# arhix52/Strelka

Measured on AMD Instinct MI355X. Metric: Mray/s, higher is better.
Workload: dtype f32; 1 GPU; kitchen stand-in (SURVEY 8d C3): 1724134 unique triangles, 2022 instances of 153 meshes, 4 rect + 1 distant light, 60/25/10/5 % diffuse/glossy/metal/glass; resolution=1920x1080, bounces=4, spp=64, tile=32, world_size=1, parallelism=single GPU, rays_per_frame=839862650

## Files before the change

strelka_amd/build.py:

```python
import os
import subprocess

HERE = os.path.dirname(os.path.abspath(__file__))
ROOT = os.path.dirname(HERE)
LIB = os.environ.get("SKH_LIB") or os.path.join(HERE, "libstrelka_hip.so")
SRC = os.path.join(HERE, "csrc", "strelka_hip.hip")
DEPS = [SRC] + [os.path.join(HERE, "csrc", f) for f in ("skh_device.h", "skh_bvh.h", "skh_env.h", "skh_emit.h", "skh_blend.h", "skh_adapt.h", "skh_aov.h", "skh_denoise.h", "skh_temporal.h", "skh_variance.h", "skh_lshape.h", "skh_kernels.h", "skh_shade_body.inc", "skh_trace_body.inc", "skh_libm.h", "skh_host.h", "skh_stale.h", "skh_accel.inc", "skh_probes.inc")] + [
    os.path.join(ROOT, "include", "strelka_hip.h"), os.path.abspath(__file__)]
FLAGS = ["-O3", "--offload-arch=gfx950", "-ffp-contract=off", "-fno-slp-vectorize", "-mllvm", "-amdgpu-sched-strategy=max-ilp",
         "-fPIC", "-shared", "-std=c++17"]


def hipcc():
    for c in (os.environ.get("HIPCC"), "/opt/rocm/bin/hipcc", "hipcc"):
        if c and (os.path.isabs(c) and os.path.exists(c) or not os.path.isabs(c)):
            return c
    return "hipcc"


def needs_build():
    if os.environ.get("SKH_LIB") and os.path.exists(LIB):
        return False
    return not os.path.exists(LIB) or any(os.path.getmtime(d) > os.path.getmtime(LIB) for d in DEPS)


def build_variant(out_path, defines, verbose=False):
    cmd = [hipcc()] + FLAGS + ["-D" + d for d in defines] + ["-o", out_path, SRC]
    if verbose:
        print(" ".join(cmd))
    subprocess.check_call(cmd)
    return out_path


def build(force=False, verbose=False):
    if not force and not needs_build():
        return LIB
    import fcntl

    with open(LIB + ".lock", "w") as lock:
        fcntl.flock(lock, fcntl.LOCK_EX)
        try:
            if force or needs_build():
                tmp = "%s.tmp.%d" % (LIB, os.getpid())
                cmd = [hipcc()] + FLAGS + ["-o", tmp, SRC]
                if verbose:
                    print(" ".join(cmd))
                subprocess.check_call(cmd)
                os.replace(tmp, LIB)
        finally:
            fcntl.flock(lock, fcntl.LOCK_UN)
    return LIB


HOST_DIR = os.path.join(HERE, "host")
HOST_LIB = os.path.join(HOST_DIR, "liboka_hip.so")
HOST_TEST = os.path.join(HOST_DIR, "host_test")


def build_host(force=False, verbose=False):
    build(force=False, verbose=verbose)
# ... 40 lines not shown
```

strelka_amd/csrc/skh_host.h:

```cpp
#pragma once
#include "../../include/strelka_hip.h"
#include "skh_kernels.h"
#include "skh_stale.h"

#include <string>
#include <utility>
#include <vector>

typedef struct ncclComm* ncclComm_t;
using namespace skh;

namespace
{
struct DevBuf
{
    void* p = nullptr;
    size_t bytes = 0;
    DevBuf() = default;
    DevBuf(const DevBuf&) = delete;
    DevBuf& operator=(const DevBuf&) = delete;
    DevBuf(DevBuf&& o) noexcept : p(o.p), bytes(o.bytes)
    {
        o.p = nullptr;
        o.bytes = 0;
    }
    DevBuf& operator=(DevBuf&& o) noexcept
    {
        if (this != &o)
        {
            reset();
            p = o.p, bytes = o.bytes;
            o.p = nullptr, o.bytes = 0;
        }
        return *this;
    }
    ~DevBuf()
    {
        reset();
    }
    void reset()
    {
        if (p)
            (void)hipFree(p);
        p = nullptr;
        bytes = 0;
    }
    template <typename T>
    T* as() const
    {
        return reinterpret_cast<T*>(p);
    }
};

enum KernelClass
{
// ... 32 lines not shown
        uint32_t* hOverflow = nullptr;
        std::string err;
    } dev;

    struct MultiGpu
    {
        ncclComm_t comm = nullptr;
        int world = 1, rank = 0;
        DevBuf dTileSend, dScatterXY;
    } multi;

    struct Scene
    {
        std::vector<skh_mesh> meshes;
        std::vector<skh_curve> curves;
        std::vector<uint32_t> curveVertexCounts;
        std::vector<skh_instance> instances;
        std::vector<int32_t> lightTypes;
        uint32_t nVerts = 0, nIndices = 0, nPoints = 0, nInstances = 0, nLights = 0, nMaterials = 0;
        DevBuf dVerts, dIndices, dMeshes, dPoints, dRadii, dInstances, dLights, dMaterials, dHairConst;
        uint64_t geomSig = 0, curveSig = 0;
        DevBuf dTexels, dTexDesc;
        uint32_t nTextures = 0;
        bool hasHairMaterial = false;
    } scene;

    struct Options
    {
        bool countTraversal = false, timing = false;
        int overlap = 1;
        uint32_t speculateAsync = 1;
        uint32_t speculateGrow = 2;
        uint32_t speculateMax = 8;
        uint32_t envNee = 1, emitNee = 1;
        uint32_t cutoutRounds = 8;
        uint32_t aovBand = 1u << 22;
        int32_t fetchChunk = -1;
        uint32_t wavesPerCU = 28;
        uint32_t wavesPerCUShadow = 28;
        uint32_t wavesPerCUShadowWorld = 32;
        uint32_t wavesPerCUWorld = 32;
        uint32_t smallWavesClosest = 0, smallWavesShadow = 0;
        uint32_t fetchMinClosestSmall = 48;
        uint32_t smallWavesFirst = 0, smallWavesLast = 0;
        int tailSplit = 1;
        uint32_t fetchMinClosest = 32 , fetchMinShadow = 48;
        bool fetchMinClosestSet = false;
        uint32_t curveFetchMinClosest = 16, curveFetchMinShadow = 16 , curveNodeBreakClosest = 20, curveNodeBreakShadow = 20;
        uint32_t nodeBreakClosest = 32, nodeBreakShadow = 28;
        uint32_t worldCurveMin = 32;
        uint32_t curveMin = 48;
        uint32_t leafMin = 16;
        uint32_t subframeBatch = 0;
        bool worldKernel = true;
        uint32_t reinsertRounds = 8;
        uint32_t reinsertCurveRounds = 4;
        uint32_t reinsertMinSize = 0;
        uint32_t plocTop = 0;
        bool tightInstanceBoxes = true;
        uint32_t curveLeaf = 1;
        uint32_t splitPairs = 0;
        uint32_t curveMerge = 1;
        uint32_t curveSegNode = 0;
        uint32_t curveStrandMajor = 0;
        uint32_t curveSplit = 4;
        uint32_t tlasBuild = 1;
        uint32_t tlasOpen = 1;
        uint32_t bakeWorld = 4, bakeSmallTris = 64, bakeBudgetMTris = 64;
        uint32_t mortonBits = 10;
        uint32_t leafLines = 0;
        uint32_t mergeLightProxies = 0;
        int32_t directRecords = -1;
        uint32_t compactHits = 1;
        uint32_t leafMaxTris = 2;
        uint32_t buildQuality = 1;
    } opt;

    struct Accel
    {
        bool built = false;
        DevBuf dTriNodes, dTris, dSegNodes, dSegs, dTlasNodes, dTlasInst, dDevInst, dTravInst;
        DevBuf dShadeTris, dShadeInst;
        DevBuf dCurveSegBase, dSegStartAll;
        int tlasRoot = SKH_REF_INVALID;
        int worldRoot = SKH_REF_INVALID, lightRoot = SKH_REF_INVALID;
        uint32_t nTris = 0, nSegs = 0;
        uint32_t nTriSlots = 0;
        uint32_t hierNodes = 0;
        uint32_t numTlasLeaves = 0;
        uint32_t curveSplitBuilt = 1;
        uint32_t numWorldCurves = 0;
        int worldCurveRoot[SKH_WORLD_CURVES];
        uint32_t worldCurveInst[SKH_WORLD_CURVES];
        uint32_t worldCurveMerged = 0;
        uint32_t worldCurveIdentLast = 0;
        uint32_t numMergedCurveInst = 0;
        std::vector<uint8_t> baked;
        uint32_t nBakedTris = 0, nBakedInst = 0;
        LightBox lightBox = { { -INFINITY, -INFINITY, -INFINITY }, { INFINITY, INFINITY, INFINITY } };
        uint32_t nShadeRecords = 0;
        uint32_t directRecords = 1;
        uint32_t hitPrimRange = 0;
        skh_build_info buildInfo = {};
        double msBuild = 0.0;
        bool refitReady = false;
        DevBuf dTriOrder, dTriMeshK, dTriLocalK, dWInstK, dWFirstK, dTriNodeBox;
// ... 17 lines not shown
        std::vector<uint32_t> tlasLevelStart;
    } accel;

    struct Environment
    {
        DevBuf dTexels, dColCdf, dRowCdf;
        uint32_t w = 0, h = 0;
        float scale[3] = { 1.0f, 1.0f, 1.0f }, w2e[9] = { 1.0f, 0.0f, 0.0f, 0.0f, 1.0f, 0.0f, 0.0f, 0.0f, 1.0f };
        double sumW = 0.0, msBuild = 0.0;
    } env;

    struct Emitters
    {
        std::vector<float> emission;
        bool stale = false;
        DevBuf dEntries, dCdf, dGuide, dLe, dInstOffset;
        uint32_t count = 0, instances = 0, guideBits = 0;
        double sumW = 0.0, msBuild = 0.0;
    } emit;

    struct MaterialTextures
    {
        std::vector<skh_material_textures> table;
        DevBuf dTable;
    } mtex;

    struct Cut
    {
        std::vector<skh_material_cutout> cutouts;
        DevBuf dCutouts, dStats, dQ[2], dHits, dShadowQ[2], dShadowHits[2];
        bool stale = false;
        uint32_t activeMaterials = 0, instances = 0;
        std::vector<skh_material_blend> blends;
        DevBuf dBlend;
        uint32_t blendActiveMaterials = 0, blendInstances = 0;
    } cut;

    struct LightShapes
    {
        std::vector<skh_light_shape> table;
        DevBuf dTable;
        bool stale = false;
        uint32_t discs = 0, cones = 0;
    } lshape;

    struct Frame
    {
        uint32_t width = 0, height = 0, tileSize = 32, tileShift = 5, numTiles = 0, numSlots = 0;
        std::vector<uint32_t> tileXY;
        bool customTiles = false;
        DevBuf dTileXY, dAccum, dDiffuse, dSpecular, dDiffCnt, dSpecCnt, dSums, dPath, dRayQ[2], dHits, dShadowQ, dContrib, dCounts, dOvf, dOvf2, dScratchImage;
        DevBuf dRaygenBase;
        uint32_t raygenBlocksPerSub = 0, raygenValidPerSub = 0;
        std::vector<uint32_t> chunkValid;
        uint32_t queueConstBits[2] = { 0, 0 };
        bool queueConstFilled = false;
        uint32_t batchCapacity = 1;
        uint32_t queueRegion = 64;
        uint32_t traceBlocks = 0;
    } frame;

    struct Speculation
    {
        bool valid = false;
        skh_frame_params params;
        uint32_t count = 0, consumed = 0, lastBatch = 1, streak = 0;
        skh_frame_params last;
        bool haveLast = false;
        uint64_t passRadiance = 0, passShadow = 0;
        uint32_t buf = 0;
        bool nextInFlight = false;
        skh_frame_params nextParams;
        uint32_t nextCount = 0;
        unsigned long long statsMark[2] = { 0, 0 };
        DevBuf dPathB;
        uint32_t pathBStride = 0;
        uint64_t discardedRadiance = 0, discardedShadow = 0;
        uint32_t discardedSubframes = 0;
    } spec;

    struct Adaptive
    {
        bool on = false;
        skh_adaptive cfg = {};
        bool ready = false;
        uint32_t delivered = 0;
        uint32_t checks = 0, activeTiles = 0, raygenValid = 0;
        uint64_t pixelObs = 0, pixelObsSaved = 0;
        std::vector<uint32_t> frozenAt;
        DevBuf dTileXYRender, dRaygenBaseRender, dState, dTileQ, dFrozenAt;
    } adapt;

    struct Timing
    {
        std::vector<TimedSpan> spans;
        std::vector<hipEvent_t> eventPool;
        size_t eventsUsed = 0;
        double msClass[KC_COUNT] = { 0, 0, 0, 0, 0, 0, 0 };
        uint32_t launches[KC_COUNT] = { 0, 0, 0, 0, 0, 0, 0 };
        DevBuf dStats;
        uint32_t stackOverflows = 0;
    } timing;

    struct Aov
    {
        skh_aov_info info = {};
    } aov;

    struct Denoiser
    {
        DevBuf dColor[2], dG0, dG1;
        skh_denoise_info info = {};
    } dn;

    struct Temporal
    {
        skh_temporal_info info = {};
    } tp;

    struct Moments
    {
        skh_moments_info info = {};
    } mo;
    struct VarianceDenoiser
    {
        skh_vdenoise_info info = {};
    } vd;
};

static inline void touched(skh_context* c, skh_stale::Input in)
{
    using namespace skh_stale;
    bool* flag[D_COUNT] = {};
    flag[D_ACCEL_BUILT] = &c->accel.built, flag[D_REFIT_READY] = &c->accel.refitReady, flag[D_UPDATE_READY] = &c->accel.updateReady;
    flag[D_VERTS_EDITED] = &c->accel.vertsEdited, flag[D_CURVE_POINTS_EDITED] = &c->accel.curvePointsEdited;
    flag[D_EMIT_STALE] = &c->emit.stale, flag[D_CUT_STALE] = &c->cut.stale, flag[D_LSHAPE_STALE] = &c->lshape.stale;
    apply(in, flag);
}

#define SKH_TRY(ctx, expr)                                                                                              \
// ... 41 lines not shown
```

strelka_amd/csrc/skh_kernels.h:

```cpp
#pragma once
#include "skh_bvh.h"
#include "skh_env.h"
#include "skh_emit.h"
#include "skh_blend.h"

namespace skh
{

struct DevInstance
{
    float w2o[12];
    int rootRef;
    uint32_t mask;
    uint32_t type;
    uint32_t pad;
};
struct HostInstance
{
    float o2w[12];
    uint32_t type, geom, material, light;
};

#define SKH_WORLD_CURVES 2
#define SKH_SEG_STRIDE 8
// ... 503 lines not shown
    __syncthreads();
    if (threadIdx.x == 0)
    {
        uint32_t tot = 0;
        for (uint32_t w = 0; w < nw; ++w)
        {
            const uint32_t cnt = s_wave[w];
            s_wave[w] = tot;
            tot += cnt;
        }
        s_wave[SKH_COMPACT_MAX_WAVES] = tot ? atomicAdd(counter, tot) : 0u;
    }
    __syncthreads();
    const uint32_t r = s_wave[SKH_COMPACT_MAX_WAVES] + s_wave[wave] + rank_below(m);
    __syncthreads();
    return r;
}
SKH_DI void block_compact2(bool emitA, uint32_t* counterA, bool emitB, uint32_t* counterB, uint32_t* s_wave2, uint32_t& ia, uint32_t& ib)
{
    const uint32_t lane = threadIdx.x & 63u, wave = threadIdx.x >> 6, nw = blockDim.x >> 6;
    const unsigned long long ma = __ballot(emitA), mb = __ballot(emitB);
    uint32_t* sa = s_wave2;
    uint32_t* sb = s_wave2 + SKH_COMPACT_MAX_WAVES + 1;
    if (lane == 0)
    {
        sa[wave] = (uint32_t)__popcll(ma);
        sb[wave] = (uint32_t)__popcll(mb);
    }
    __syncthreads();
    if (threadIdx.x == 0 || threadIdx.x == 64)
    {
        uint32_t* sw = threadIdx.x == 0 ? sa : sb;
        uint32_t tot = 0;
        for (uint32_t w = 0; w < nw; ++w)
        {
            const uint32_t cnt = sw[w];
            sw[w] = tot;
            tot += cnt;
        }
        sw[SKH_COMPACT_MAX_WAVES] = tot ? atomicAdd(threadIdx.x == 0 ? counterA : counterB, tot) : 0u;
    }
    if (nw == 1 && threadIdx.x == 0)
    {
        uint32_t tot = sb[0];
        sb[0] = 0;
        sb[SKH_COMPACT_MAX_WAVES] = tot ? atomicAdd(counterB, tot) : 0u;
    }
    __syncthreads();
    ia = sa[SKH_COMPACT_MAX_WAVES] + sa[wave] + rank_below(ma);
    ib = sb[SKH_COMPACT_MAX_WAVES] + sb[wave] + rank_below(mb);
}

__global__ void __launch_bounds__(512) k_raygen(FrameP fp, const uint32_t* __restrict__ tileXY, uint32_t sampleOffset, RayQ rq,
                                               uint32_t* __restrict__ counter, PathS ps, const uint32_t* __restrict__ blockBase,
                                               uint32_t blocksPerSub, uint32_t validPerSub)
{
    __shared__ uint32_t s_wave[SKH_COMPACT_MAX_WAVES + 1];
    const uint32_t sub = blockIdx.x / blocksPerSub, bi = blockIdx.x - sub * blocksPerSub;
    const uint32_t slot = bi * blockDim.x + threadIdx.x;
    const uint32_t path = sub * fp.numSlots + slot;
    uint32_t px = 0, py = 0;
    const bool active = sub < fp.batch && slot < fp.numSlots && slot_to_pixel(fp, tileXY, slot, px, py);
    v3 o = mk3(0.0f), d = mk3(0.0f);
    if (active)
    {
        const Sampler s = init_sampler(px, py, fp.subframeIndex + sampleOffset + sub, fp.sppTotal, 52u);
        generate_camera_ray(px, py, fp.width, fp.height, fp.clipToView, fp.viewToWorld, sampler_random(s, DIM_PIXEL_X),
                            sampler_random(s, DIM_PIXEL_Y), o, d);
        ps.rad()[path] = make_float4(0.0f, 0.0f, 0.0f, 0.0f);
        reinterpret_cast<uint32_t*>(ps.base)[path + 7 * (size_t)ps.stride] = 0u;
    }
    const uint32_t lane = threadIdx.x & 63u, wave = threadIdx.x >> 6;
    const unsigned long long m = __ballot(active);
    if (lane == 0)
        s_wave[wave] = (uint32_t)__popcll(m);
    __syncthreads();
    uint32_t before = 0;
    for (uint32_t w = 0; w < wave; ++w)
        before += s_wave[w];
    const uint32_t dense = sub * validPerSub + blockBase[bi] + before + rank_below(m);
    const uint32_t total = validPerSub * fp.batch;
    const uint32_t per = (((total + SKH_SHARDS - 1u) / SKH_SHARDS) + 63u) & ~63u;
    const uint32_t shard = per ? dense / per : 0u;
    const uint32_t idx = shard * rq.region + (dense - shard * per);
    if (blockIdx.x == 0 && threadIdx.x < SKH_SHARDS)
        counter[threadIdx.x * SKH_COUNT_STRIDE] = min(per, total - min(total, threadIdx.x * per));
    if (active)
    {
        rq.plane(0)[idx] = o.x;
        rq.plane(1)[idx] = o.y;
        rq.plane(2)[idx] = o.z;
        rq.plane(3)[idx] = d.x;
        rq.plane(4)[idx] = d.y;
        rq.plane(5)[idx] = d.z;
        rq.ids()[idx] = path;
    }
}

__global__ void __launch_bounds__(256) k_gather_shade_tris(const uint8_t* __restrict__ verts, const uint32_t* __restrict__ indices,
                                                          const uint4* __restrict__ meshes, const uint32_t* __restrict__ meshTriBase,
                                                          uint32_t nMeshes, uint32_t nTris, float4* __restrict__ out)
{
    const uint32_t g = blockIdx.x * blockDim.x + threadIdx.x;
    if (g >= nTris)
        return;
    uint32_t lo = 0, hi = nMeshes;
    while (hi - lo > 1u)
    {
        const uint32_t mid = (lo + hi) >> 1;
        if (meshTriBase[mid] <= g)
            lo = mid;
        else
            hi = mid;
    }
    const uint4 me = meshes[lo];
    const uint32_t t = g - meshTriBase[lo];
    float4 v0[3], v1[3];
#pragma unroll
    for (uint32_t k = 0; k < 3u; ++k)
    {
        const uint32_t idx = indices[me.x + 3u * t + k];
        const float4* v = reinterpret_cast<const float4*>(verts + (size_t)(me.z + idx) * 32);
        v0[k] = v[0], v1[k] = v[1];
    }
    float4* o = out + 6 * (size_t)g;
#pragma unroll
    for (uint32_t k = 0; k < 3u; ++k)
        o[k] = make_float4(v0[k].x, v0[k].y, v0[k].z, v1[k].x);
    o[3] = make_float4(v0[0].w, v0[1].w, v0[2].w, v1[0].y);
    o[4] = make_float4(v1[1].y, v1[2].y, 0.0f, 0.0f);
    o[5] = make_float4(0.0f, 0.0f, 0.0f, 0.0f);
}

// ... 926 lines not shown
```

strelka_amd/csrc/strelka_hip.hip:

```cpp
#include "../../include/strelka_hip.h"
#include "skh_kernels.h"

#include <dlfcn.h>
typedef struct ncclComm* ncclComm_t;
typedef struct
{
    char internal[128];
} ncclUniqueId;
typedef enum
{
    ncclSuccess = 0
} ncclResult_t;
typedef enum
{
    ncclFloat = 7
} ncclDataType_t;

#include <algorithm>
#include <chrono>
#include <cmath>
#include <cstdio>
#include <cstring>
#include <mutex>
#include <string>
// ... 468 lines not shown
{
    const uint32_t nMeshes = (uint32_t)c->scene.meshes.size();
    std::vector<uint32_t> base(nMeshes + 1u, 0u);
    uint64_t total = 0;
    for (uint32_t m = 0; m < nMeshes; ++m)
    {
        total += c->scene.meshes[m].index_count / 3u;
        base[m + 1] = (uint32_t)std::min<uint64_t>(total, 0xffffffffull);
    }
    const uint32_t nTris = base[nMeshes];
    c->accel.nShadeRecords = nTris;
    if (total >= SKH_PRIM_DIRECT)
    {
        c->dev.err = "skh_build_accel: more than 2^31 - 1 triangles (the primitive word of a hit keeps its top bit for SKH_PRIM_DIRECT)";
        return SKH_INVALID_ARGUMENT;
    }
    SKH_CHECK(dev_alloc(c, c->accel.dShadeTris, std::max<size_t>(96, (size_t)nTris * 96)));
    if (nTris)
    {
        DevBuf dBase;
        SKH_CHECK(dev_upload(c, dBase, base.data(), sizeof(uint32_t) * base.size()));
        k_gather_shade_tris<<<(nTris + 255u) / 256u, 256, 0, c->dev.stream>>>(c->scene.dVerts.as<uint8_t>(), c->scene.dIndices.as<uint32_t>(), c->scene.dMeshes.as<uint4>(),
                                                                         dBase.as<uint32_t>(), nMeshes, nTris, c->accel.dShadeTris.as<float4>());
        SKH_TRY(c, hipStreamSynchronize(c->dev.stream));
    }
    std::vector<skh_instance> inst = c->scene.instances;
    for (skh_instance& i : inst)
        if (i.type == SKH_INSTANCE_MESH)
            i.light_id = i.geom_id < nMeshes ? base[i.geom_id] : 0u;
    if (inst.empty())
        inst.resize(1);
    return dev_upload(c, c->accel.dShadeInst, inst.data(), sizeof(skh_instance) * inst.size());
}

#include "skh_accel.inc"


static size_t frame_count_words(const skh_context* c);

static void raygen_tables(const skh_context* c, const uint32_t* frozenAt, std::vector<uint32_t>& base, uint32_t& total)
{
    const uint32_t blocks = (c->frame.numSlots + 511u) / 512u, chunks = (uint32_t)c->frame.chunkValid.size(), shift2 = 2 * c->frame.tileShift;
    base.assign(std::max(1u, blocks), 0u);
    total = 0;
    for (uint32_t b = 0; b < blocks; ++b)
    {
        base[b] = total;
        for (uint32_t j = b * 8u; j < std::min(chunks, (b + 1) * 8u); ++j)
            if (!frozenAt || frozenAt[(j * 64u) >> shift2] == 0u)
                total += c->frame.chunkValid[j];
    }
}

static skh_status alloc_frame(skh_context* c)
{
    const uint32_t T = c->frame.tileSize;
    if (!c->frame.customTiles)
    {
        c->frame.tileXY.clear();
        for (uint32_t y = 0; y < c->frame.height; y += T)
            for (uint32_t x = 0; x < c->frame.width; x += T)
            {
                c->frame.tileXY.push_back(x);
                c->frame.tileXY.push_back(y);
            }
    }
    c->frame.numTiles = (uint32_t)(c->frame.tileXY.size() / 2);
    c->frame.numSlots = c->frame.numTiles * T * T;
    c->frame.batchCapacity = c->opt.subframeBatch ? c->opt.subframeBatch : std::min(64u, std::max(1u, (1u << 27) / std::max(1u, c->frame.numSlots)));
    const size_t N1 = std::max(1u, c->frame.numSlots);
    const size_t N = N1 * c->frame.batchCapacity;
    c->frame.queueRegion = (uint32_t)((((N + SKH_SHARDS - 1) / SKH_SHARDS) + 63) & ~(size_t)63);
    const size_t NQ = (size_t)SKH_SHARDS * c->frame.queueRegion;
    SKH_CHECK(dev_upload(c, c->frame.dTileXY, c->frame.tileXY.data(), sizeof(uint32_t) * c->frame.tileXY.size()));
    {
        auto compact = [](uint32_t x) {
            x &= 0x55555555u;
            x = (x ^ (x >> 1)) & 0x33333333u;
            x = (x ^ (x >> 2)) & 0x0f0f0f0fu;
            x = (x ^ (x >> 4)) & 0x00ff00ffu;
            x = (x ^ (x >> 8)) & 0x0000ffffu;
            return x;
        };
        const uint32_t shift2 = 2 * c->frame.tileShift, mask = (1u << shift2) - 1u;
        c->frame.chunkValid.assign(c->frame.numSlots / 64u, 0u);
        for (uint32_t j = 0; j < c->frame.numSlots / 64u; ++j)
        {
            const uint32_t tile = (j * 64u) >> shift2, m = (j * 64u) & mask;
            const uint32_t x0 = c->frame.tileXY[2 * tile] + compact(m), y0 = c->frame.tileXY[2 * tile + 1] + compact(m >> 1);
            uint32_t n = 0;
            for (uint32_t k = 0; k < 64u; ++k)
                n += (x0 + compact(k) < c->frame.width && y0 + compact(k >> 1) < c->frame.height) ? 1u : 0u;
            c->frame.chunkValid[j] = n;
        }
        std::vector<uint32_t> base;
        raygen_tables(c, nullptr, base, c->frame.raygenValidPerSub);
        c->frame.raygenBlocksPerSub = (uint32_t)((c->frame.numSlots + 511u) / 512u);
        SKH_CHECK(dev_upload(c, c->frame.dRaygenBase, base.data(), sizeof(uint32_t) * base.size()));
    }
    c->adapt.ready = false;
    SKH_CHECK(dev_alloc(c, c->frame.dAccum, sizeof(float4) * N1));
    SKH_CHECK(dev_alloc(c, c->frame.dDiffuse, sizeof(float4) * N1));
    SKH_CHECK(dev_alloc(c, c->frame.dSpecular, sizeof(float4) * N1));
    SKH_CHECK(dev_alloc(c, c->frame.dDiffCnt, sizeof(uint16_t) * N1));
    SKH_CHECK(dev_alloc(c, c->frame.dSpecCnt, sizeof(uint16_t) * N1));
    SKH_CHECK(dev_alloc(c, c->frame.dSums, sizeof(float) * 11 * N1));
    SKH_CHECK(dev_alloc(c, c->frame.dPath, sizeof(float) * SKH_PATH_FLOATS * N));
    SKH_CHECK(dev_alloc(c, c->frame.dRayQ[0], sizeof(float) * 9 * NQ));
    SKH_CHECK(dev_alloc(c, c->frame.dRayQ[1], sizeof(float) * 9 * NQ));
// ... 972 lines not shown
    if (!a || !std::isfinite(a->threshold) || a->threshold < 0.0f || !std::isfinite(a->dark_level) || !(a->dark_level > 0.0f) || a->min_samples < 2u ||
        a->interval < 1u || a->reserved[0] || a->reserved[1] || a->reserved[2] || a->reserved[3])
        return SKH_INVALID_ARGUMENT;
    return SKH_OK;
}

skh_status skh_set_adaptive(skh_context* c, const skh_adaptive* a)
{
    if (!c || (a && skh_adaptive_check(a) != SKH_OK))
    {
        if (c)
            c->dev.err = "skh_set_adaptive: threshold finite and >= 0, dark_level finite and > 0, min_samples >= 2, interval >= 1, reserved words 0";
        return SKH_INVALID_ARGUMENT;
    }
    (void)hipSetDevice(c->dev.device);
    spec_drop(c);
    c->adapt.on = a != nullptr;
    if (a)
        c->adapt.cfg = *a;
    else
    {
        SKH_TRY(c, hipStreamSynchronize(c->dev.stream));
        c->adapt = skh_context::Adaptive();
    }
    return SKH_OK;
}

static inline bool adapt_applies(const skh_context* c, const skh_frame_params& p)
{
    return c->adapt.on && p.enable_accumulation != 0 && p.debug == 0;
}

static skh_status adapt_prepare(skh_context* c, const skh_frame_params& p)
{
    skh_context::Adaptive& ad = c->adapt;
    if (ad.ready && p.subframe_index != 0)
        return SKH_OK;
    const size_t N1 = std::max(1u, c->frame.numSlots), nt = std::max(1u, c->frame.numTiles);
    const size_t baseBytes = sizeof(uint32_t) * std::max(1u, c->frame.raygenBlocksPerSub);
    SKH_CHECK(dev_alloc(c, c->adapt.dTileXYRender, sizeof(uint32_t) * 2 * nt));
    SKH_CHECK(dev_alloc(c, c->adapt.dRaygenBaseRender, baseBytes));
    SKH_CHECK(dev_alloc(c, c->adapt.dState, sizeof(float4) * N1));
    SKH_CHECK(dev_alloc(c, c->adapt.dTileQ, sizeof(float) * nt));
    SKH_CHECK(dev_alloc(c, c->adapt.dFrozenAt, sizeof(uint32_t) * nt));
    SKH_TRY(c, hipMemcpyAsync(c->adapt.dTileXYRender.p, c->frame.dTileXY.p, sizeof(uint32_t) * 2 * c->frame.numTiles, hipMemcpyDeviceToDevice, c->dev.stream));
    SKH_TRY(c, hipMemcpyAsync(c->adapt.dRaygenBaseRender.p, c->frame.dRaygenBase.p, baseBytes, hipMemcpyDeviceToDevice, c->dev.stream));
    SKH_TRY(c, hipMemsetAsync(c->adapt.dState.p, 0, sizeof(float4) * N1, c->dev.stream));
    SKH_TRY(c, hipMemsetAsync(c->adapt.dTileQ.p, 0, sizeof(float) * nt, c->dev.stream));
    SKH_TRY(c, hipMemsetAsync(c->adapt.dFrozenAt.p, 0, sizeof(uint32_t) * nt, c->dev.stream));
    ad.frozenAt.assign(c->frame.numTiles, 0u);
    ad.delivered = ad.checks = 0;
    ad.activeTiles = c->frame.numTiles;
    ad.raygenValid = c->frame.raygenValidPerSub;
    ad.pixelObs = ad.pixelObsSaved = 0;
    ad.ready = true;
    return SKH_OK;
}

static inline uint32_t adapt_to_next_check(const skh_context* c)
{
    const skh_context::Adaptive& ad = c->adapt;
    if (ad.delivered < ad.cfg.min_samples)
        return ad.cfg.min_samples - ad.delivered;
    return ad.cfg.interval - (ad.delivered - ad.cfg.min_samples) % ad.cfg.interval;
}

static void frame_geometry(const skh_context* c, FrameP& fp)
{
    fp.width = c->frame.width, fp.height = c->frame.height, fp.tileSize = c->frame.tileSize, fp.tileShift = c->frame.tileShift, fp.numTiles = c->frame.numTiles, fp.numSlots = c->frame.numSlots;
}

static FrameP adapt_frame(const skh_context* c, const skh_frame_params& p)
{
    FrameP fp;
    memset(&fp, 0, sizeof(fp));
    memcpy(fp.exposure, p.exposure, sizeof(fp.exposure));
    frame_geometry(c, fp);
    return fp;
}

static skh_status adapt_after_pass(skh_context* c, const skh_frame_params& p, uint32_t launches)
{
    skh_context::Adaptive& ad = c->adapt;
    ad.delivered += launches;
    ad.pixelObs += (uint64_t)ad.raygenValid * launches;
    ad.pixelObsSaved += (uint64_t)(c->frame.raygenValidPerSub - ad.raygenValid) * launches;
    if (ad.delivered < ad.cfg.min_samples || (ad.delivered - ad.cfg.min_samples) % ad.cfg.interval != 0u || c->frame.numTiles == 0u)
        return SKH_OK;
    const float thr2 = ad.cfg.threshold * ad.cfg.threshold;
    {
        SpanGuard g(c, KC_ACCUM);
        k_adapt_tiles<<<c->frame.numTiles, 256, 0, c->dev.stream>>>(adapt_frame(c, p), c->adapt.dTileXYRender.as<uint32_t>(), c->adapt.dState.as<float4>(), ad.delivered, thr2,
                                                          ad.cfg.dark_level, c->adapt.dTileQ.as<float>(), c->adapt.dFrozenAt.as<uint32_t>());
    }
    ad.checks++;
    SKH_TRY(c, hipMemcpyAsync(ad.frozenAt.data(), c->adapt.dFrozenAt.p, sizeof(uint32_t) * c->frame.numTiles, hipMemcpyDeviceToHost, c->dev.stream));
    SKH_TRY(c, hipStreamSynchronize(c->dev.stream));
    uint32_t active = 0;
    for (uint32_t t = 0; t < c->frame.numTiles; ++t)
        active += ad.frozenAt[t] == 0u ? 1u : 0u;
    if (active != ad.activeTiles)
    {
        std::vector<uint32_t> base;
        raygen_tables(c, ad.frozenAt.data(), base, ad.raygenValid);
        SKH_TRY(c, hipMemcpyAsync(c->adapt.dRaygenBaseRender.p, base.data(), sizeof(uint32_t) * base.size(), hipMemcpyHostToDevice, c->dev.stream));
        SKH_TRY(c, hipStreamSynchronize(c->dev.stream));
        ad.activeTiles = active;
    }
    return SKH_OK;
}

static void adapt_fill(skh_context* c, const skh_frame_params& p, void* d_image)
{
    if (!d_image || c->adapt.activeTiles == c->frame.numTiles || c->frame.numSlots == 0u)
        return;
    SpanGuard g(c, KC_ACCUM);
    k_adapt_fill<<<(c->frame.numSlots + 255) / 256, 256, 0, c->dev.stream>>>(adapt_frame(c, p), c->frame.dTileXY.as<uint32_t>(), c->adapt.dFrozenAt.as<uint32_t>(),
                                                                 c->frame.dAccum.as<float4>(), reinterpret_cast<float4*>(d_image));
}

skh_status skh_get_adaptive_info(skh_context* c, skh_adaptive_info* out)
{
    if (!c || !out)
        return SKH_INVALID_ARGUMENT;
    const skh_context::Adaptive& ad = c->adapt;
    memset(out, 0, sizeof(*out));
    out->enabled = ad.on ? 1u : 0u;
    out->tiles = c->frame.numTiles;
    out->active_tiles = c->frame.numTiles;
    if (!ad.on || !ad.ready)
        return SKH_OK;
    out->active_tiles = ad.activeTiles;
    out->checks = ad.checks;
    uint32_t lo = 0xffffffffu, hi = 0;
    for (uint32_t t = 0; t < c->frame.numTiles; ++t)
    {
        const uint32_t n = ad.frozenAt[t] ? ad.frozenAt[t] : ad.delivered;
        lo = std::min(lo, n), hi = std::max(hi, n);
    }
    out->min_observations = c->frame.numTiles ? lo : 0u;
    out->max_observations = hi;
    out->pixel_observations = ad.pixelObs;
    out->pixel_observations_saved = ad.pixelObsSaved;
    return SKH_OK;
}

struct RenderPlan
{
    uint32_t batch = 1;
    bool trace = true;
    uint32_t finalFirst = 0, finalCount = 0xffffffffu;
    uint32_t pathSel = 0;
    bool finalize = true;
    hipStream_t finStream = nullptr;
    bool adaptive = false;
};

struct RenderPass
{
    FrameP fp;
// ... 116 lines not shown
        t.smallGrid = smallGrids ? ((b + 1 == rp.rounds && (c->opt.smallWavesLast || (!c->opt.smallWavesShadow && !c->accel.nSegs))) ? (c->opt.smallWavesLast ? c->opt.smallWavesLast : 20u) : c->opt.smallWavesShadow ? c->opt.smallWavesShadow : (c->accel.nSegs ? 16u : 12u)) * (uint32_t)c->dev.numCUs : 0u;
        const CutRounds cr{ { rp.cutSQ[0], rp.cutSQ[1] }, rp.cutSH0, rp.cutSH1, nullptr, rp.cutOn ? words + c->opt.cutoutRounds * SKH_CUT_WORDS : nullptr, rp.NP, blp };
        trace_step(c, rp.sc, t, true, rp.cutOn ? &cr : nullptr);
    }
    if (rp.useOverlap)
        (void)hipEventRecord(c->dev.evShadow, sst);
}

static void render_accumulate(skh_context* c, const RenderPass& rp, const RenderPlan& plan, bool oneSampleDirect, void* d_image)
{
    if (!plan.finalize)
        return;
    const uint32_t gridSlots = (c->frame.numSlots + 255) / 256;
    const bool fromPaths = plan.batch > 1 || oneSampleDirect;
    hipStream_t fs = plan.finStream ? plan.finStream : rp.st;
    {
        SpanGuard g(c, KC_ACCUM, fs);
        if (fromPaths)
            k_finalize_batch<<<gridSlots, 256, 0, fs>>>(rp.fp, rp.tiles, rp.ps, c->frame.dAccum.as<float4>(), c->frame.dDiffuse.as<float4>(), c->frame.dSpecular.as<float4>(),
                                                        c->frame.dDiffCnt.as<uint16_t>(), c->frame.dSpecCnt.as<uint16_t>(), reinterpret_cast<float4*>(d_image));
        else
            k_finalize<<<gridSlots, 256, 0, fs>>>(rp.fp, rp.tiles, c->frame.dSums.as<float>(), c->frame.dAccum.as<float4>(), c->frame.dDiffuse.as<float4>(), c->frame.dSpecular.as<float4>(),
                                                  c->frame.dDiffCnt.as<uint16_t>(), c->frame.dSpecCnt.as<uint16_t>(), reinterpret_cast<float4*>(d_image));
    }
    if (plan.adaptive)
    {
        SpanGuard g(c, KC_ACCUM, fs);
        k_adapt_moments<<<gridSlots, 256, 0, fs>>>(rp.fp, rp.tiles, rp.ps, c->frame.dSums.as<float>(), fromPaths ? 0u : 1u, c->adapt.dState.as<float4>());
    }
}

static skh_status render_one(skh_context* c, const skh_frame_params* p, const RenderPlan& plan, void* d_image)
{
    if (p->max_depth > 128 || p->samples_this_launch == 0)
    {
        c->dev.err = "skh_render_subframe: max_depth must be <= 128 (MAX_BOUNCES, RandomSampler.h:35) and samples_this_launch >= 1";
        return SKH_INVALID_ARGUMENT;
    }
    RenderPass rp;
    hipStream_t st = rp.st = c->dev.stream;
    const FrameP& fp = rp.fp = frame_params(c, p, plan);
    const uint32_t batch = plan.batch;
    rp.sc = make_dev_scene(c);
    rp.envp = make_env(c);
    rp.emitp = make_emit(c);
    rp.mtexp = make_mtex(c);
    rp.lshp = make_lshape(c);
    const uint32_t N = c->frame.numSlots * c->frame.batchCapacity;
    const uint32_t NQ = SKH_SHARDS * c->frame.queueRegion;
    const uint32_t NP = rp.NP = c->frame.numSlots * batch;
    if (NP == 0)
        return SKH_OK;
    rp.tiles = plan.adaptive ? c->adapt.dTileXYRender.as<uint32_t>() : c->frame.dTileXY.as<uint32_t>();
    const uint32_t* raygenBase = plan.adaptive ? c->adapt.dRaygenBaseRender.as<uint32_t>() : c->frame.dRaygenBase.as<uint32_t>();
    const uint32_t raygenValid = plan.adaptive ? c->adapt.raygenValid : c->frame.raygenValidPerSub;
    rp.ps = PathS{ plan.pathSel ? c->spec.dPathB.as<float>() : c->frame.dPath.as<float>(), plan.pathSel ? c->spec.pathBStride : N };
    const auto queue = [&](const DevBuf& b) { return RayQ{ b.as<float>(), NQ, c->frame.queueRegion }; };
    rp.rq[0] = queue(c->frame.dRayQ[0]), rp.rq[1] = queue(c->frame.dRayQ[1]), rp.shq = queue(c->frame.dShadowQ);
    HitQ hq{ c->frame.dHits.as<float>(), NQ };
    {
        const bool worldKernels = trace_build(c, false) >= TB_WORLD;
        const uint32_t range = std::max(1u, c->accel.hitPrimRange);
        uint32_t B = 1;
        while (B < 31u && (1u << B) < range)
            ++B;
        hq.primBits = (c->opt.compactHits && worldKernels && c->accel.nShadeRecords != 0u && (uint64_t)c->scene.nInstances <= (1ull << (32u - B)) - 1ull && (1ull << B) >= range) ? B : 0u;
        hq.direct = c->accel.directRecords;
        hq.recClamp = c->accel.nShadeRecords ? c->accel.nShadeRecords - 1u : 0u;
    }
    rp.hq = hq;
    fill_queue_constants(c, rp);
    uint32_t* counts = rp.counts = c->frame.dCounts.as<uint32_t>();
    const uint32_t QW = rp.QW = SKH_COUNT_STRIDE * SKH_SHARDS;
    rp.fetch = counts + QW * 2 * SKH_MAX_LAUNCH_ROUNDS;
    rp.smallPass = NP <= (1u << 23) || c->opt.overlap == 2;
    rp.useOverlap = (c->opt.overlap == 2 || (c->opt.overlap == 1 && NP <= (1u << 25))) && fp.debug != 1;
    const uint32_t rounds = rp.rounds = fp.maxDepth;
    const bool cutOn = rp.cutOn = cut_stage_on(c);
    rp.cutBounceWords = 2u * c->opt.cutoutRounds * SKH_CUT_WORDS;
    rp.cutWords = rp.fetch + 16 * SKH_FETCH_STRIDE * (rounds + 1);
    rp.cutQ[0] = queue(c->cut.dQ[0]), rp.cutQ[1] = queue(c->cut.dQ[1]), rp.cutSQ[0] = queue(c->cut.dShadowQ[0]), rp.cutSQ[1] = queue(c->cut.dShadowQ[1]);
    rp.cutH = rp.cutSH0 = rp.cutSH1 = hq;
    rp.cutH.base = c->cut.dHits.as<float>(), rp.cutSH0.base = c->cut.dShadowHits[0].as<float>(), rp.cutSH1.base = c->cut.dShadowHits[1].as<float>();
    rp.blp = make_blend(c);
    rp.blp.tileXY = rp.tiles, rp.blp.sppTotal = fp.sppTotal, rp.blp.numSlots = fp.numSlots, rp.blp.tileShift = fp.tileShift;
    rp.blp.contrib = c->frame.dContrib.as<float4>();
    rp.split = c->opt.tailSplit < 0 && rp.smallPass && NP >= (1u << 17);
    const bool oneSampleDirect = batch == 1 && fp.samplesThisLaunch == 1 && plan.finalize && fp.finalFirst == 0 && fp.finalCount == 1;
    for (uint32_t s = 0; plan.trace && s < fp.samplesThisLaunch; ++s)
    {
        SKH_TRY(c, hipMemsetAsync(counts, 0, sizeof(uint32_t) * (QW * 2 * SKH_MAX_LAUNCH_ROUNDS + 16 * SKH_FETCH_STRIDE * (rounds + 1) + (size_t)(cutOn ? rounds : 0u) * rp.cutBounceWords), st));
        rp.blp.sampleBase = fp.subframeIndex + s;
        {
            SpanGuard g(c, KC_RAYGEN);
            k_raygen<<<c->frame.raygenBlocksPerSub * fp.batch, 512, 0, st>>>(fp, rp.tiles, s, rp.rq[0], counts, rp.ps, raygenBase, c->frame.raygenBlocksPerSub, raygenValid);
        }
        for (uint32_t b = 0; b < rounds; ++b)
        {
            render_bounce(c, rp, s, b);
            if (fp.debug == 1)
                break;
        }
        if (rp.useOverlap)
            (void)hipStreamWaitEvent(st, c->dev.evShadow, 0);
        {
            SpanGuard g(c, KC_ACCUM);
            k_add_stats<<<1, 64, 0, st>>>(counts, rounds, c->timing.dStats.as<StatsDev>());
            if (batch == 1 && !oneSampleDirect)
                k_collect<<<(c->frame.numSlots + 255) / 256, 256, 0, st>>>(fp, rp.tiles, s, rp.ps, c->frame.dSums.as<float>());
        }
    }
    render_accumulate(c, rp, plan, oneSampleDirect, d_image);
    hipError_t e = hipGetLastError();
    if (e != hipSuccess)
    {
        c->dev.err = std::string("render launch: ") + hipGetErrorString(e);
        return SKH_FAIL;
    }
    return SKH_OK;
}

skh_status skh_render_subframes(skh_context* c, const skh_frame_params* params, uint32_t n_subframes, void* d_image)
{
    if (!c || !params)
        return SKH_INVALID_ARGUMENT;
    (void)hipSetDevice(c->dev.device);
    if (c->frame.width == 0)
    {
        c->dev.err = "skh_render_subframe: call skh_resize first";
        return SKH_INVALID_ARGUMENT;
    }
    skh_status s = ensure_ready(c);
    if (s != SKH_OK)
        return s;
    if (n_subframes != 1)
        spec_drop(c, false, true);
    else
        spec_drop(c, true);
    skh_frame_params p = *params;
    const uint32_t cap = (p.samples_this_launch == 1 && p.debug != 1) ? c->frame.batchCapacity : 1u;
    const bool adaptive = adapt_applies(c, p) && n_subframes != 0u;
    if (adaptive && (s = adapt_prepare(c, p)) != SKH_OK)
        return s;
    for (uint32_t k = 0; k < n_subframes;)
    {
        if (adaptive && c->adapt.activeTiles == 0u)
        {
            c->adapt.pixelObsSaved += (uint64_t)c->frame.raygenValidPerSub * (n_subframes - k);
// ... 1083 lines not shown
{
    if (!c || !out)
        return SKH_INVALID_ARGUMENT;
    *out = c->vd.info;
    out->scratch_bytes = denoise_scratch_bytes(c);
    return SKH_OK;
}

enum OptEffect
{
    OPT_NONE,
    OPT_REBUILD,
    OPT_FRAME
};
struct OptRow
{
    const char* name;
    int64_t lo, hi;
    OptEffect effect;
    void (*store)(skh_context*, int64_t);
    bool needsSegNode = false;
    bool skh_context::Options::*counters = nullptr;
};
static const int64_t kOptMin = INT64_MIN, kOptMax = INT64_MAX;
#define OPT_U32(field) [](skh_context* c, int64_t v) { c->opt.field = (uint32_t)v; }
#define OPT_I32(field) [](skh_context* c, int64_t v) { c->opt.field = (int32_t)v; }
#define OPT_FLAG(field) [](skh_context* c, int64_t v) { c->opt.field = v != 0; }
static const OptRow kOptions[] = {
    { "count_traversal", kOptMin, kOptMax, OPT_NONE, OPT_FLAG(countTraversal), false, &skh_context::Options::countTraversal },
    { "timing", kOptMin, kOptMax, OPT_NONE, OPT_FLAG(timing), false, &skh_context::Options::timing },
    { "fetch_min_closest", 1, 64, OPT_NONE, [](skh_context* c, int64_t v) { c->opt.fetchMinClosestSet = true, c->opt.fetchMinClosest = c->opt.curveFetchMinClosest = (uint32_t)v; } },
    { "fetch_min_shadow", 1, 64, OPT_NONE, [](skh_context* c, int64_t v) { c->opt.fetchMinShadow = c->opt.curveFetchMinShadow = (uint32_t)v; } },
    { "node_break_closest", 0, 64, OPT_NONE, [](skh_context* c, int64_t v) { c->opt.nodeBreakClosest = c->opt.curveNodeBreakClosest = (uint32_t)v; } },
    { "node_break_shadow", 0, 64, OPT_NONE, [](skh_context* c, int64_t v) { c->opt.nodeBreakShadow = c->opt.curveNodeBreakShadow = (uint32_t)v; } },
    { "curve_min", 1, 64, OPT_NONE, [](skh_context* c, int64_t v) { c->opt.curveMin = c->opt.worldCurveMin = (uint32_t)v; } },
    { "fetch_min_closest_small", 1, 64, OPT_NONE, OPT_U32(fetchMinClosestSmall) },
    { "fetch_chunk", -1, 4096, OPT_NONE, OPT_I32(fetchChunk) },
    { "leaf_min", 0, 64, OPT_NONE, OPT_U32(leafMin) },
    { "overlap", 0, 2, OPT_NONE, OPT_I32(overlap) },
    { "tail_split", -1, 2, OPT_NONE, OPT_I32(tailSplit) },
    { "small_waves_first", 0, 64, OPT_NONE, OPT_U32(smallWavesFirst) },
    { "small_waves_last", 0, 64, OPT_NONE, OPT_U32(smallWavesLast) },
    { "small_waves_closest", 0, 64, OPT_NONE, OPT_U32(smallWavesClosest) },
    { "small_waves_shadow", 0, 64, OPT_NONE, OPT_U32(smallWavesShadow) },
    { "env_nee", 0, 1, OPT_NONE, OPT_U32(envNee) },
    { "emit_nee", 0, 1, OPT_NONE, OPT_U32(emitNee) },
    { "cutout_rounds", 1, 32, OPT_NONE, OPT_U32(cutoutRounds) },
    { "aov_band", 64, 1 << 26, OPT_NONE, OPT_U32(aovBand) },
    { "speculate", 0, 64, OPT_NONE, OPT_U32(speculateMax) },
    { "speculate_grow", 2, 64, OPT_NONE, OPT_U32(speculateGrow) },
    { "speculate_async", 0, 1, OPT_NONE, [](skh_context* c, int64_t v) { spec_drop(c), c->opt.speculateAsync = (uint32_t)v; } },
    { "world_kernel", kOptMin, kOptMax, OPT_NONE, OPT_FLAG(worldKernel) },
    { "subframe_batch", 0, 64, OPT_FRAME, OPT_U32(subframeBatch) },
    { "waves_per_cu", 1, 32, OPT_FRAME, OPT_U32(wavesPerCU) },
    { "waves_per_cu_shadow", 1, 32, OPT_FRAME, OPT_U32(wavesPerCUShadow) },
    { "waves_per_cu_world", 1, 32, OPT_FRAME, OPT_U32(wavesPerCUWorld) },
    { "waves_per_cu_shadow_world", 1, 32, OPT_FRAME, OPT_U32(wavesPerCUShadowWorld) },
    { "compact_hits", 0, 1, OPT_REBUILD, OPT_U32(compactHits) },
    { "direct_records", -1, 1, OPT_REBUILD, OPT_I32(directRecords) },
    { "merge_light_proxies", 0, 1, OPT_REBUILD, OPT_U32(mergeLightProxies) },
    { "tight_instance_boxes", kOptMin, kOptMax, OPT_REBUILD, OPT_FLAG(tightInstanceBoxes) },
    { "curve_leaf", 1, 4, OPT_REBUILD, OPT_U32(curveLeaf) },
    { "split_pairs", 0, 1000, OPT_REBUILD, OPT_U32(splitPairs) },
    { "curve_merge", 0, 1, OPT_REBUILD, OPT_U32(curveMerge) },
    { "curve_segnode", 0, 1, OPT_REBUILD, OPT_U32(curveSegNode), true },
    { "curve_strand_major", 0, 1, OPT_REBUILD, OPT_U32(curveStrandMajor), true },
    { "curve_split", 1, 8, OPT_REBUILD, OPT_U32(curveSplit) },
    { "tlas_build", 0, 2, OPT_REBUILD, OPT_U32(tlasBuild) },
    { "tlas_open", 0, 64, OPT_REBUILD, OPT_U32(tlasOpen) },
    { "bake_world", 0, 4, OPT_REBUILD, OPT_U32(bakeWorld) },
    { "bake_budget_mtris", 0, 100, OPT_REBUILD, OPT_U32(bakeBudgetMTris) },
    { "bake_small_tris", 0, 1 << 20, OPT_REBUILD, OPT_U32(bakeSmallTris) },
    { "morton_bits", 4, 21, OPT_REBUILD, OPT_U32(mortonBits) },
    { "leaf_lines", 0, 1, OPT_REBUILD, OPT_U32(leafLines) },
    { "leaf_max_tris", 1, 8, OPT_REBUILD, OPT_U32(leafMaxTris) },
    { "build_quality", kOptMin, kOptMax, OPT_REBUILD, OPT_FLAG(buildQuality) },
    { "reinsert_rounds", 0, 64, OPT_REBUILD, OPT_U32(reinsertRounds) },
    { "reinsert_curve_rounds", 0, 64, OPT_REBUILD, OPT_U32(reinsertCurveRounds) },
    { "reinsert_min_size", 0, 1 << 24, OPT_REBUILD, OPT_U32(reinsertMinSize) },
    { "ploc_top", 0, kOptMax, OPT_REBUILD, OPT_U32(plocTop) },
};
#undef OPT_U32
#undef OPT_I32
#undef OPT_FLAG

skh_status skh_set_option(skh_context* c, const char* name, int64_t value)
{
    if (!c || !name)
        return SKH_INVALID_ARGUMENT;
    const OptRow* row = nullptr;
    for (const OptRow& r : kOptions)
        if (strcmp(r.name, name) == 0)
            row = &r;
    if (!row || !row->counters)
        spec_drop(c);
    else if (c->opt.*(row->counters) != (value != 0))
        spec_drop(c, true);
    if (!row)
    {
        c->dev.err = std::string("skh_set_option: unknown option ") + name;
        return SKH_INVALID_ARGUMENT;
    }
    if (value < row->lo || value > row->hi || (row->needsSegNode && value == 1 && !SKH_SEGNODE))
        return SKH_INVALID_ARGUMENT;
    row->store(c, value);
    if (row->effect == OPT_REBUILD)
// ... 180 lines not shown
```

Measured before the change: 6423 Mray/s.

## Reorder raygen queue slots by Morton-sorted cells interleaved across shards

Adds a host-built table mapping each raygen wave (or block cell) to a queue base and per-subframe stride. Cells are sorted along a Morton curve over pixel origins and dealt round-robin across shards, so that with batched subframes the same pixel region's samples sit next to each other in the ray queue. The goal is more coherent rays within waves, improving BVH traversal cache locality. In exchange it adds host table construction and uploads, cached per batch and generation, plus an extra indirection and changed launch geometry in raygen.

```diff
diff --git a/strelka_amd/build.py b/strelka_amd/build.py
--- a/strelka_amd/build.py
+++ b/strelka_amd/build.py
@@ -5,7 +5,7 @@
 ROOT = os.path.dirname(HERE)
 LIB = os.environ.get("SKH_LIB") or os.path.join(HERE, "libstrelka_hip.so")
 SRC = os.path.join(HERE, "csrc", "strelka_hip.hip")
-DEPS = [SRC] + [os.path.join(HERE, "csrc", f) for f in ("skh_device.h", "skh_bvh.h", "skh_env.h", "skh_emit.h", "skh_blend.h", "skh_adapt.h", "skh_aov.h", "skh_denoise.h", "skh_temporal.h", "skh_variance.h", "skh_lshape.h", "skh_kernels.h", "skh_shade_body.inc", "skh_trace_body.inc", "skh_libm.h", "skh_host.h", "skh_stale.h", "skh_accel.inc", "skh_probes.inc")] + [
+DEPS = [SRC] + [os.path.join(HERE, "csrc", f) for f in ("skh_device.h", "skh_bvh.h", "skh_env.h", "skh_emit.h", "skh_blend.h", "skh_adapt.h", "skh_aov.h", "skh_denoise.h", "skh_temporal.h", "skh_variance.h", "skh_lshape.h", "skh_kernels.h", "skh_shade_body.inc", "skh_trace_body.inc", "skh_libm.h", "skh_host.h", "skh_stale.h", "skh_order.h", "skh_accel.inc", "skh_probes.inc")] + [
     os.path.join(ROOT, "include", "strelka_hip.h"), os.path.abspath(__file__)]
 FLAGS = ["-O3", "--offload-arch=gfx950", "-ffp-contract=off", "-fno-slp-vectorize", "-mllvm", "-amdgpu-sched-strategy=max-ilp",
          "-fPIC", "-shared", "-std=c++17"]
diff --git a/strelka_amd/csrc/skh_host.h b/strelka_amd/csrc/skh_host.h
--- a/strelka_amd/csrc/skh_host.h
+++ b/strelka_amd/csrc/skh_host.h
@@ -1,6 +1,7 @@
 #pragma once
 #include "../../include/strelka_hip.h"
 #include "skh_kernels.h"
+#include "skh_order.h"
 #include "skh_stale.h"
 
 #include <string>
@@ -139,6 +140,8 @@
         uint32_t curveMin = 48;
         uint32_t leafMin = 16;
         uint32_t subframeBatch = 0;
+        uint32_t queueOrder = 1;
+        int32_t cellBlocks = 0;
         bool worldKernel = true;
         uint32_t reinsertRounds = 8;
         uint32_t reinsertCurveRounds = 4;
@@ -262,6 +265,15 @@
         DevBuf dTileXY, dAccum, dDiffuse, dSpecular, dDiffCnt, dSpecCnt, dSums, dPath, dRayQ[2], dHits, dShadowQ, dContrib, dCounts, dOvf, dOvf2, dScratchImage;
         DevBuf dRaygenBase;
         uint32_t raygenBlocksPerSub = 0, raygenValidPerSub = 0;
+        struct CellTables
+        {
+            uint32_t batch = 0, gen = 0;
+            int32_t cellBlocks = 0;
+            bool adaptive = false;
+            DevBuf dQBase, dSubStride;
+        };
+        std::vector<CellTables> cellTables;
+        uint32_t cellTablesNext = 0;
         std::vector<uint32_t> chunkValid;
         uint32_t queueConstBits[2] = { 0, 0 };
         bool queueConstFilled = false;
@@ -296,6 +308,7 @@
         bool ready = false;
         uint32_t delivered = 0;
         uint32_t checks = 0, activeTiles = 0, raygenValid = 0;
+        uint32_t orderGen = 0;
         uint64_t pixelObs = 0, pixelObsSaved = 0;
         std::vector<uint32_t> frozenAt;
         DevBuf dTileXYRender, dRaygenBaseRender, dState, dTileQ, dFrozenAt;
diff --git a/strelka_amd/csrc/skh_kernels.h b/strelka_amd/csrc/skh_kernels.h
--- a/strelka_amd/csrc/skh_kernels.h
+++ b/strelka_amd/csrc/skh_kernels.h
@@ -579,11 +579,14 @@
 }
 
 __global__ void __launch_bounds__(512) k_raygen(FrameP fp, const uint32_t* __restrict__ tileXY, uint32_t sampleOffset, RayQ rq,
-                                               uint32_t* __restrict__ counter, PathS ps, const uint32_t* __restrict__ blockBase,
-                                               uint32_t blocksPerSub, uint32_t validPerSub)
+                                               uint32_t* __restrict__ counter, PathS ps, const uint32_t* __restrict__ qBase,
+                                               const uint32_t* __restrict__ subStride, uint32_t blocksPerSub, uint32_t validPerSub,
+                                               uint32_t launchCell, uint32_t perWave)
 {
     __shared__ uint32_t s_wave[SKH_COMPACT_MAX_WAVES + 1];
-    const uint32_t sub = blockIdx.x / blocksPerSub, bi = blockIdx.x - sub * blocksPerSub;
+    const uint32_t span = launchCell * fp.batch, lc = blockIdx.x / span, inSpan = blockIdx.x - lc * span;
+    const uint32_t nb = min(launchCell, blocksPerSub - lc * launchCell);
+    const uint32_t sub = inSpan / nb, bi = lc * launchCell + (inSpan - sub * nb);
     const uint32_t slot = bi * blockDim.x + threadIdx.x;
     const uint32_t path = sub * fp.numSlots + slot;
     uint32_t px = 0, py = 0;
@@ -603,9 +606,10 @@
         s_wave[wave] = (uint32_t)__popcll(m);
     __syncthreads();
     uint32_t before = 0;
-    for (uint32_t w = 0; w < wave; ++w)
+    for (uint32_t w = 0; w < wave && !perWave; ++w)
         before += s_wave[w];
-    const uint32_t dense = sub * validPerSub + blockBase[bi] + before + rank_below(m);
+    const uint32_t u = perWave ? bi * 8u + wave : bi;
+    const uint32_t dense = qBase[u] + sub * (subStride ? subStride[u] : validPerSub) + before + rank_below(m);
     const uint32_t total = validPerSub * fp.batch;
     const uint32_t per = (((total + SKH_SHARDS - 1u) / SKH_SHARDS) + 63u) & ~63u;
     const uint32_t shard = per ? dense / per : 0u;
diff --git a/strelka_amd/csrc/skh_order.h b/strelka_amd/csrc/skh_order.h
--- /dev/null
+++ b/strelka_amd/csrc/skh_order.h
@@ -0,0 +1,106 @@
+#pragma once
+#include <algorithm>
+#include <cstdint>
+#include <vector>
+
+namespace skh_order
+{
+constexpr uint32_t kNoCell = 0xffffffffu;
+
+struct Tables
+{
+    std::vector<uint32_t> qBase, subStride;
+    uint32_t validPerSub = 0;
+    std::vector<uint32_t> curvePos, runStart;
+};
+
+inline uint32_t even_bits(uint32_t x)
+{
+    x &= 0x55555555u;
+    x = (x ^ (x >> 1)) & 0x33333333u;
+    x = (x ^ (x >> 2)) & 0x0f0f0f0fu;
+    x = (x ^ (x >> 4)) & 0x00ff00ffu;
+    x = (x ^ (x >> 8)) & 0x0000ffffu;
+    return x;
+}
+
+inline uint64_t spread_bits(uint32_t x)
+{
+    uint64_t v = x;
+    v = (v | (v << 16)) & 0x0000ffff0000ffffull;
+    v = (v | (v << 8)) & 0x00ff00ff00ff00ffull;
+    v = (v | (v << 4)) & 0x0f0f0f0f0f0f0f0full;
+    v = (v | (v << 2)) & 0x3333333333333333ull;
+    v = (v | (v << 1)) & 0x5555555555555555ull;
+    return v;
+}
+inline uint64_t morton_key(uint32_t x, uint32_t y)
+{
+    return spread_bits(x) | (spread_bits(y) << 1);
+}
+
+inline uint32_t per_shard(uint32_t total, uint32_t shards)
+{
+    return (((total + shards - 1u) / shards) + 63u) & ~63u;
+}
+
+inline void slot_order(const uint32_t* valid, uint32_t nUnits, Tables& t)
+{
+    t.qBase.assign(std::max(1u, nUnits), 0u);
+    t.curvePos.clear(), t.runStart.clear();
+    uint32_t total = 0;
+    for (uint32_t u = 0; u < nUnits; ++u)
+    {
+        t.qBase[u] = total;
+        total += valid[u];
+    }
+    t.validPerSub = total;
+    t.subStride.assign(std::max(1u, nUnits), total);
+}
+
+inline void cell_order(const uint32_t* valid, const uint32_t* originXY, uint32_t nUnits, uint32_t batch, uint32_t cellUnits, uint32_t shards, Tables& t)
+{
+    cellUnits = std::max(1u, cellUnits), shards = std::max(1u, shards);
+    const uint32_t nCells = (nUnits + cellUnits - 1u) / cellUnits;
+    std::vector<uint32_t> cellValid(nCells, 0u);
+    for (uint32_t u = 0; u < nUnits; ++u)
+        cellValid[u / cellUnits] += valid[u];
+    std::vector<uint32_t> curve;
+    for (uint32_t k = 0; k < nCells; ++k)
+        if (cellValid[k])
+            curve.push_back(k);
+    std::stable_sort(curve.begin(), curve.end(), [&](uint32_t a, uint32_t b) {
+        return morton_key(originXY[2 * (size_t)a * cellUnits], originXY[2 * (size_t)a * cellUnits + 1]) < morton_key(originXY[2 * (size_t)b * cellUnits], originXY[2 * (size_t)b * cellUnits + 1]);
+    });
+    t.curvePos.assign(nCells, kNoCell);
+    for (uint32_t i = 0; i < (uint32_t)curve.size(); ++i)
+        t.curvePos[curve[i]] = i;
+    std::vector<uint32_t> cellBase(nCells, 0u);
+    t.runStart.assign(shards + 1u, 0u);
+    uint32_t pos = 0, perSub = 0;
+    for (uint32_t g = 0; g < shards; ++g)
+    {
+        t.runStart[g] = pos;
+        for (size_t i = g; i < curve.size(); i += shards)
+        {
+            cellBase[curve[i]] = pos;
+            pos += cellValid[curve[i]] * batch;
+            perSub += cellValid[curve[i]];
+        }
+    }
+    t.runStart[shards] = pos;
+    t.validPerSub = perSub;
+    t.qBase.assign(std::max(1u, nUnits), 0u);
+    t.subStride.assign(std::max(1u, nUnits), 0u);
+    for (uint32_t k = 0; k < nCells; ++k)
+    {
+        uint32_t inCell = 0;
+        for (uint32_t u = k * cellUnits; u < std::min(nUnits, (k + 1u) * cellUnits); ++u)
+        {
+            t.qBase[u] = cellBase[k] + inCell;
+            t.subStride[u] = cellValid[k];
+            inCell += valid[u];
+        }
+    }
+}
+}
diff --git a/strelka_amd/csrc/strelka_hip.hip b/strelka_amd/csrc/strelka_hip.hip
--- a/strelka_amd/csrc/strelka_hip.hip
+++ b/strelka_amd/csrc/strelka_hip.hip
@@ -544,9 +544,74 @@
     }
 }
 
+struct RaygenOrder
+{
+    const uint32_t *qBase = nullptr, *subStride = nullptr;
+    uint32_t launchCell = 1, perWave = 0;
+};
+
+static int32_t cell_blocks(const skh_context* c)
+{
+    return c->opt.cellBlocks ? c->opt.cellBlocks : -1;
+}
+
+static skh_status raygen_order(skh_context* c, bool adaptive, uint32_t batch, RaygenOrder& out)
+{
+    skh_context::Frame& f = c->frame;
+    out = RaygenOrder{};
+    out.qBase = adaptive ? c->adapt.dRaygenBaseRender.as<uint32_t>() : f.dRaygenBase.as<uint32_t>();
+    out.launchCell = std::max(1u, f.raygenBlocksPerSub);
+    if (c->opt.queueOrder == 0u || batch <= 1u)
+        return SKH_OK;
+    const int32_t cb = cell_blocks(c);
+    const uint32_t gen = adaptive ? c->adapt.orderGen : 0u;
+    out.perWave = cb < 0 ? 1u : 0u;
+    out.launchCell = cb < 0 ? 1u : std::min((uint32_t)cb, std::max(1u, f.raygenBlocksPerSub));
+    skh_context::Frame::CellTables* e = nullptr;
+    for (skh_context::Frame::CellTables& t : f.cellTables)
+        if (t.batch == batch && t.cellBlocks == cb && t.adaptive == adaptive && t.gen == gen)
+            e = &t;
+    if (!e)
+    {
+        const uint32_t perUnit = cb < 0 ? 1u : 8u, chunks = (uint32_t)f.chunkValid.size(), shift2 = 2 * f.tileShift, mask = (1u << shift2) - 1u;
+        const uint32_t nUnits = f.raygenBlocksPerSub * (cb < 0 ? 8u : 1u);
+        const uint32_t* frozenAt = adaptive ? c->adapt.frozenAt.data() : nullptr;
+        std::vector<uint32_t> valid(nUnits, 0u), origin(2 * (size_t)nUnits, 0u);
+        for (uint32_t u = 0; u < nUnits; ++u)
+        {
+            const uint32_t j0 = u * perUnit;
+            if (j0 >= chunks)
+                continue;
+            const uint32_t tile = (j0 * 64u) >> shift2, m = (j0 * 64u) & mask;
+            origin[2 * (size_t)u] = f.tileXY[2 * tile] + skh_order::even_bits(m), origin[2 * (size_t)u + 1] = f.tileXY[2 * tile + 1] + skh_order::even_bits(m >> 1);
+            for (uint32_t j = j0; j < std::min(chunks, j0 + perUnit); ++j)
+                if (!frozenAt || frozenAt[(j * 64u) >> shift2] == 0u)
+                    valid[u] += f.chunkValid[j];
+        }
+        skh_order::Tables t;
+        skh_order::cell_order(valid.data(), origin.data(), nUnits, batch, cb < 0 ? 1u : (uint32_t)cb, SKH_SHARDS, t);
+        if (t.validPerSub != (adaptive ? c->adapt.raygenValid : f.raygenValidPerSub))
+        {
+            c->dev.err = "raygen_order: the cell order counts other slots than the slot order";
+            return SKH_FAIL;
+        }
+        if (f.cellTables.size() < 8u)
+            f.cellTables.emplace_back(), e = &f.cellTables.back();
+        else
+            e = &f.cellTables[f.cellTablesNext++ % 8u];
+        e->batch = 0;
+        SKH_CHECK(dev_upload(c, e->dQBase, t.qBase.data(), sizeof(uint32_t) * t.qBase.size()));
+        SKH_CHECK(dev_upload(c, e->dSubStride, t.subStride.data(), sizeof(uint32_t) * t.subStride.size()));
+        e->batch = batch, e->cellBlocks = cb, e->adaptive = adaptive, e->gen = gen;
+    }
+    out.qBase = e->dQBase.as<uint32_t>(), out.subStride = e->dSubStride.as<uint32_t>();
+    return SKH_OK;
+}
+
 static skh_status alloc_frame(skh_context* c)
 {
     const uint32_t T = c->frame.tileSize;
+    c->frame.cellTables.clear();
     if (!c->frame.customTiles)
     {
         c->frame.tileXY.clear();
@@ -1625,6 +1690,7 @@
     ad.delivered = ad.checks = 0;
     ad.activeTiles = c->frame.numTiles;
     ad.raygenValid = c->frame.raygenValidPerSub;
+    ad.orderGen++;
     ad.pixelObs = ad.pixelObsSaved = 0;
     ad.ready = true;
     return SKH_OK;
@@ -1679,6 +1745,7 @@
         SKH_TRY(c, hipMemcpyAsync(c->adapt.dRaygenBaseRender.p, base.data(), sizeof(uint32_t) * base.size(), hipMemcpyHostToDevice, c->dev.stream));
         SKH_TRY(c, hipStreamSynchronize(c->dev.stream));
         ad.activeTiles = active;
+        ad.orderGen++;
     }
     return SKH_OK;
 }
@@ -1901,7 +1968,9 @@
     if (NP == 0)
         return SKH_OK;
     rp.tiles = plan.adaptive ? c->adapt.dTileXYRender.as<uint32_t>() : c->frame.dTileXY.as<uint32_t>();
-    const uint32_t* raygenBase = plan.adaptive ? c->adapt.dRaygenBaseRender.as<uint32_t>() : c->frame.dRaygenBase.as<uint32_t>();
+    RaygenOrder order;
+    if (plan.trace)
+        SKH_CHECK(raygen_order(c, plan.adaptive, batch, order));
     const uint32_t raygenValid = plan.adaptive ? c->adapt.raygenValid : c->frame.raygenValidPerSub;
     rp.ps = PathS{ plan.pathSel ? c->spec.dPathB.as<float>() : c->frame.dPath.as<float>(), plan.pathSel ? c->spec.pathBStride : N };
     const auto queue = [&](const DevBuf& b) { return RayQ{ b.as<float>(), NQ, c->frame.queueRegion }; };
@@ -1942,7 +2011,9 @@
         rp.blp.sampleBase = fp.subframeIndex + s;
         {
             SpanGuard g(c, KC_RAYGEN);
-            k_raygen<<<c->frame.raygenBlocksPerSub * fp.batch, 512, 0, st>>>(fp, rp.tiles, s, rp.rq[0], counts, rp.ps, raygenBase, c->frame.raygenBlocksPerSub, raygenValid);
+            const uint32_t launchCells = (c->frame.raygenBlocksPerSub + order.launchCell - 1u) / order.launchCell;
+            k_raygen<<<launchCells * order.launchCell * fp.batch, 512, 0, st>>>(fp, rp.tiles, s, rp.rq[0], counts, rp.ps, order.qBase, order.subStride, c->frame.raygenBlocksPerSub, raygenValid,
+                                                                                 order.launchCell, order.perWave);
         }
         for (uint32_t b = 0; b < rounds; ++b)
         {
@@ -3132,6 +3203,8 @@
     { "speculate_async", 0, 1, OPT_NONE, [](skh_context* c, int64_t v) { spec_drop(c), c->opt.speculateAsync = (uint32_t)v; } },
     { "world_kernel", kOptMin, kOptMax, OPT_NONE, OPT_FLAG(worldKernel) },
     { "subframe_batch", 0, 64, OPT_FRAME, OPT_U32(subframeBatch) },
+    { "queue_order", 0, 1, OPT_NONE, OPT_U32(queueOrder) },
+    { "cell_blocks", -1, 64, OPT_NONE, OPT_I32(cellBlocks) },
     { "waves_per_cu", 1, 32, OPT_FRAME, OPT_U32(wavesPerCU) },
     { "waves_per_cu_shadow", 1, 32, OPT_FRAME, OPT_U32(wavesPerCUShadow) },
     { "waves_per_cu_world", 1, 32, OPT_FRAME, OPT_U32(wavesPerCUWorld) },
```

Result: faster. 6512 Mray/s, median of 6 (+1.4%).
